# Christina-hshi/SH-assembly

Hardware: AMD Instinct MI355X
Metric: k-mers counted/sec (whole node), CQF build, C.elegans-like k=47 (higher is better)
Workload: dtype u64

## Files before the change

sh-assembly_amd/csrc/kmer_kernels.hip:

```cpp
#include "shk_device.h"

#define SHK_SEED_A 0x3c8bfbb395c60474ULL
#define SHK_SEED_C 0x3193c18562a02b4cULL
#define SHK_SEED_G 0x20323ed082572324ULL
#define SHK_SEED_T 0x295549f54be24456ULL
#define SHK_HASH_WAVES 4
#define SHK_MAX_K 191
#define SHK_MAX_READ 65535

__device__ __forceinline__ uint64_t shk_seed_fwd(unsigned c) {
  const unsigned u = c & 0xDF;
  return (u == 'A' || c == 4) ? SHK_SEED_A : (u == 'C' || c == 7) ? SHK_SEED_C : (u == 'G' || c == 3) ? SHK_SEED_G : (u == 'T' || c == 1) ? SHK_SEED_T : 0ULL;
}
__device__ __forceinline__ uint64_t shk_seed_rc(unsigned c) {
  c &= 7;
  return c == 1 ? SHK_SEED_T : c == 3 ? SHK_SEED_G : c == 7 ? SHK_SEED_C : c == 4 ? SHK_SEED_A : 0ULL;
}

__device__ __forceinline__ uint32_t shk_nl_flags(uint32_t w) {
  uint32_t x = w ^ 0x0A0A0A0Au;
  return ~(((x & 0x7F7F7F7Fu) + 0x7F7F7F7Fu) | x | 0x7F7F7F7Fu);
}

__device__ __forceinline__ uint4 shk_unit_flags(const uint8_t *text, uint64_t a0, uint64_t u, uint64_t off,
                                                uint64_t end) {
  const uint4 v = *reinterpret_cast<const uint4 *>(text + a0 + 16 * u);
  uint32_t w[4] = {v.x, v.y, v.z, v.w};
  uint64_t b0 = a0 + 16 * u;
#pragma unroll
  for (int i = 0; i < 4; i++) {
    uint32_t f = shk_nl_flags(w[i]);
    uint64_t wb = b0 + 4 * i;
    if (wb < off || wb + 4 > end) {
#pragma unroll
      for (int j = 0; j < 4; j++)
        if (wb + j < off || wb + j >= end) f &= ~(0x80u << (8 * j));
    }
    w[i] = f;
  }
  return make_uint4(w[0], w[1], w[2], w[3]);
}

#define SHK_PARSE_SEGS 16
__device__ __forceinline__ void shk_segment_units(uint64_t nunits, unsigned seg, uint64_t *u0, uint64_t *u1) {
  const uint64_t per = (nunits + SHK_PARSE_SEGS - 1) / SHK_PARSE_SEGS;
  *u0 = per * seg < nunits ? per * seg : nunits;
  *u1 = *u0 + per < nunits ? *u0 + per : nunits;
}

__global__ void k_count_lines(const uint8_t *text, const uint64_t *chunk_off, const uint64_t *chunk_len,
                              uint64_t *nlines_seg) {
  __shared__ uint64_t scratch[SHK_MAX_WAVES + 1];
  const unsigned c = blockIdx.x / SHK_PARSE_SEGS, seg = blockIdx.x % SHK_PARSE_SEGS;
  const uint64_t off = chunk_off[c], end = off + chunk_len[c];
  const uint64_t a0 = off & ~15ULL;
  const uint64_t nunits = (end - a0 + 15) / 16;
  uint64_t u0, u1;
  shk_segment_units(nunits, seg, &u0, &u1);
  uint64_t cnt = 0;
  for (uint64_t u = u0 + threadIdx.x; u < u1; u += blockDim.x) {
    uint4 f = shk_unit_flags(text, a0, u, off, end);
    cnt += __popc(f.x) + __popc(f.y) + __popc(f.z) + __popc(f.w);
  }
  uint64_t tot = shk_block_sum64(cnt, scratch);
  if (threadIdx.x == 0) nlines_seg[blockIdx.x] = tot;
}

__global__ void k_scan_chunks(uint64_t *nlines_seg, unsigned nchunks, uint64_t *reads_base, uint64_t *nreads_total) {
  __shared__ uint64_t scratch[SHK_MAX_WAVES + 1];
  __shared__ uint64_t carry_s;
  if (threadIdx.x == 0) carry_s = 0;
  __syncthreads();
  for (unsigned base = 0; base < nchunks; base += blockDim.x) {
    unsigned c = base + threadIdx.x;
    uint64_t nl = 0;
    if (c < nchunks)
      for (unsigned sg = 0; sg < SHK_PARSE_SEGS; sg++) {
        const uint64_t v = nlines_seg[(uint64_t)c * SHK_PARSE_SEGS + sg];
        nlines_seg[(uint64_t)c * SHK_PARSE_SEGS + sg] = nl;
        nl += v;
      }
    uint64_t v = c < nchunks ? (nl + 2) / 4 : 0;
    uint64_t tot;
    uint64_t ex = shk_block_exscan64(v, &tot, scratch);
    uint64_t carry = carry_s;
    if (c < nchunks) reads_base[c] = carry + ex;
    __syncthreads();
    if (threadIdx.x == 0) carry_s = carry + tot;
    __syncthreads();
  }
  if (threadIdx.x == 0) {
    reads_base[nchunks] = carry_s;
    *nreads_total = carry_s;
  }
}

__global__ void k_emit_reads(const uint8_t *text, const uint64_t *chunk_off, const uint64_t *chunk_len,
                             const uint64_t *reads_base, const uint64_t *line_base_seg, uint64_t *rd_start, uint64_t *rd_end,
                             uint16_t *rd_chunk) {
  __shared__ uint32_t scratch[SHK_MAX_WAVES + 1];
  __shared__ uint64_t line_carry;
  const unsigned c = blockIdx.x / SHK_PARSE_SEGS, seg = blockIdx.x % SHK_PARSE_SEGS;
  const uint64_t off = chunk_off[c], end = off + chunk_len[c];
  const uint64_t a0 = off & ~15ULL;
  const uint64_t nunits = (end - a0 + 15) / 16;
  uint64_t u0, u1;
  shk_segment_units(nunits, seg, &u0, &u1);
  const uint64_t rbase = reads_base[c], nreads = reads_base[c + 1] - rbase;
  if (threadIdx.x == 0) line_carry = line_base_seg[blockIdx.x];
  __syncthreads();
  for (uint64_t ub = u0; ub < u1; ub += blockDim.x) {
    uint64_t u = ub + threadIdx.x;
    uint4 f = make_uint4(0, 0, 0, 0);
    if (u < u1) f = shk_unit_flags(text, a0, u, off, end);
    uint32_t n = __popc(f.x) + __popc(f.y) + __popc(f.z) + __popc(f.w);
    uint32_t tot;
    uint32_t ex = shk_block_exscan(n, &tot, scratch);
    uint64_t line = line_carry + ex;
    if (n) {
      uint32_t w[4] = {f.x, f.y, f.z, f.w};
#pragma unroll
      for (int i = 0; i < 4; i++) {
        uint32_t m = w[i];
        while (m) {
          int bit = __ffs(m) - 1;
          m &= m - 1;
          uint64_t pos = a0 + 16 * u + 4 * i + (bit >> 3);
          uint64_t rd = line >> 2;
          if (rd < nreads) {
            if ((line & 3) == 0) { rd_start[rbase + rd] = pos + 1; rd_chunk[rbase + rd] = (uint16_t)c; }
            else if ((line & 3) == 1) rd_end[rbase + rd] = pos;
          }
          line++;
        }
      }
    }
    __syncthreads();
    if (threadIdx.x == 0) line_carry += tot;
    __syncthreads();
  }
}

__device__ __forceinline__ uint32_t shk_segment_end(const uint8_t *rd, uint32_t len, uint32_t s, uint32_t k) {
  const unsigned lane = shk_lane();
  for (uint32_t base = (s + k) & ~63u; base < len; base += 64) {
    uint32_t pos = base + lane;
    bool isN = pos >= s + k && pos < len && rd[pos] == 'N';
    unsigned long long m = __ballot(isN);
    if (m) return base + (uint32_t)(__ffsll((long long)m) - 1);
  }
  return len;
}

__device__ __forceinline__ void shk_read_bytes(const uint8_t *text, uint64_t st, uint64_t en, unsigned lane, uint32_t c[4]) {
  const uint64_t len = en > st ? en - st : 0;
#pragma unroll
  for (int t = 0; t < 4; t++) {
    const uint32_t pos = (uint32_t)t * 64 + lane;
    c[t] = pos < len ? text[st + pos] : 0u;
  }
}
__device__ __forceinline__ void shk_read_masks(const uint32_t c[4], unsigned long long nm[4]) {
#pragma unroll
  for (int t = 0; t < 4; t++) nm[t] = __ballot(c[t] == 'N');
}
__device__ __forceinline__ uint32_t shk_segment_end_pre(const unsigned long long nm[4], const uint8_t *rd, uint32_t len,
                                                        uint32_t s, uint32_t k) {
  if (len > 256) return shk_segment_end(rd, len, s, k);
  const uint32_t from = s + k;
#pragma unroll
  for (int t = 0; t < 4; t++) {
    if ((uint32_t)t < (from >> 6)) continue;
    unsigned long long m = nm[t];
    if ((uint32_t)t == (from >> 6)) m &= ~0ULL << (from & 63);
    if (m) return (uint32_t)t * 64 + (uint32_t)(__ffsll((long long)m) - 1);
  }
  return len;
}

__device__ __forceinline__ uint32_t shk_bytes_below(uint32_t n) { return n >= 4 ? 0xFFFFFFFFu : ((1u << (8 * n)) - 1u); }
__global__ void k_count_keys(const uint8_t *text, const uint64_t *rd_start, const uint64_t *rd_end,
                             const uint64_t *nreads_p, uint32_t k, uint32_t *nkeys, uint32_t *err) {
  const uint64_t nreads = *nreads_p;
  const uint64_t stride = (uint64_t)gridDim.x * blockDim.x;
  for (uint64_t r = (uint64_t)blockIdx.x * blockDim.x + threadIdx.x; r < nreads; r += stride) {
    const uint64_t st = rd_start[r], en = rd_end[r];
    uint32_t cnt = 0;
    if (en - st > SHK_MAX_READ) atomicOr(err, SHK_E_BAD_FASTQ);
    else if (en - st >= k) {
      const uint32_t len = (uint32_t)(en - st);
      const uint8_t *rd = text + st;
      const uint64_t a = st + k, e = en;
      uint32_t any = 0;
      for (uint64_t u = a & ~15ULL; u < e; u += 16) {
        const uint4 v = *reinterpret_cast<const uint4 *>(text + u);
        const uint32_t w[4] = {v.x, v.y, v.z, v.w};
#pragma unroll
        for (int i = 0; i < 4; i++) {
          const uint64_t b = u + 4 * i;
          const uint32_t lo = a > b ? (uint32_t)(a - b > 4 ? 4 : a - b) : 0u;
          const uint32_t hi = e > b ? (uint32_t)(e - b > 4 ? 4 : e - b) : 0u;
          const uint32_t valid = shk_bytes_below(hi) & ~shk_bytes_below(lo);
          const uint32_t x = (w[i] ^ 0x4E4E4E4Eu) | ~valid;
          any |= (x - 0x01010101u) & ~x & 0x80808080u;
        }
      }
      if (!any) cnt = len - k + 1;
      else {
        uint32_t s0 = 0;
        while (len >= s0 + k) {
          uint32_t e0 = s0 + k;
          while (e0 < len && rd[e0] != 'N') e0++;
          cnt += e0 - s0 - k + 1;
          if (e0 == len) break;
          s0 = e0 + 1;
        }
      }
    }
    nkeys[r] = cnt;
  }
}

__global__ void k_hash_reads(const uint8_t *text, const uint64_t *rd_start, const uint64_t *rd_end,
// ... 101 lines not shown
```

sh-assembly_amd/csrc/shk_api.hip:

```cpp
#include "../../include/shk.h"
#include <thread>

#include <hip/hip_runtime.h>
#include <math.h>
#include <stdio.h>
#include <stdlib.h>
#include <string.h>
#include <vector>
#include <string>
#include <algorithm>
#include <unordered_set>
#include <unordered_map>

#include "kmer_kernels.hip"
#include "roll_kernels.hip"
#include "partition_kernels.hip"
#include "cqf_kernels.hip"
#include "merge2_kernels.hip"
#include "walk_kernels.hip"
#include "unitig_kernels.hip"

#define SHK_SLACK 256

enum {
  KP_COUNT_LINES, KP_SCAN_CHUNKS, KP_EMIT_READS, KP_COUNT_KEYS, KP_HASH, KP_SCAN, KP_RP_PREP, KP_RP_HIST,
  KP_RP_SCATTER, KP_MERGE_SUM, KP_REGION_SCAN, KP_MERGE_WRITE, KP_MERGE_SPILL, KP_PLACE, KP_MARKS, KP_LOOKUP, KP_WALK, KP_UG_WALK, KP_UG_FINISH, KP_MERGE_FUSED, KP_MERGE_SAMPLE, KP_MISC, KP_ROLL_HIST, KP_ROLL_SCATTER, KP_PACK, KP_RP_SLOTS, KP_RP_SCATTER_NARROW, KP_SPECTRUM, KP_JOIN, KP_N
};
static const char *kp_names[KP_N] = {
  "k_count_lines", "k_scan_chunks", "k_emit_reads", "k_count_keys", "k_hash_reads", "k_scan_*", "k_rp_prep",
  "k_rp_hist", "k_rp_scatter", "k_region_merge<summary>", "k_region_scan", "k_region_merge<write>",
  "k_region_merge<spill>", "k_region_place", "k_denoise_marks", "k_lookup", "k_extend_forward+k_select_seeds", "k_ug_walk", "k_ug_check/emit/median/links", "k_region_merge<fused>", "k_region_merge<sample>", "misc", "k_roll_hist", "k_roll_scatter", "k_pack_reads", "k_rp_slot_cursors", "k_rp_scatter<narrow>", "k_region_spectrum", "k_region_join"};

struct PendingEvent { int id; hipEvent_t a, b; };

#define SHK_SCALAR_WORDS 64
enum ShkDevSlot {
  DS_NREADS = 0,
  DS_NWORDS = 1,
  DS_SCAN_TOTAL = 2,
  DS_MARKS = 3,
  DS_MAX_COUNT = 4,
  DS_DUMP_STOP = 5,
  DS_JOIN_STOP = 6,
  DS_JOIN_ACC = 7,
  DS_WALK_IN = 8,
  DS_WALK_OUT = 10,
  DS_SPECTRUM = 12,
  DS_STAMPS = 16,
  DS_PAIR_LEN = 40,
  DS_PAIR_BASE = 42,
  DS_EXTENT = 46,
  DS_END = 48
};
enum ShkHostSlot {
  HP_COUNTERS = 0,
  HP_SPECTRUM = 8,
  HP_ERR = 40,
  HP_NREADS = 41,
  HP_NWORDS = 42,
  HP_NWORDS_IN = 43,
  HP_FREE_PTR = 44,
  HP_TOTAL = 45,
  HP_AUX = 46,
  HP_MARKS = 47,
  HP_IFIN = 48,
  HP_IFIRST = 49,
  HP_WALK_IN = 50,
  HP_WALK_OUT = 52,
  HP_PAIR = 56,
  HP_END = 62
};
enum { CNT_NEWD, CNT_ADDED, CNT_REMOVED, CNT_ADDED_BEFORE };
static_assert(HP_COUNTERS + SHK_NCOUNTERS <= HP_ERR, "the counters mirror ends before the error word");
static_assert(HP_COUNTERS + SHK_NCOUNTERS <= HP_SPECTRUM && DS_SPECTRUM + (int)SHK_SPEC_WORDS <= DS_STAMPS, "the spectrum's totals have four words of their own");
static_assert(DS_END <= SHK_SCALAR_WORDS && HP_END <= SHK_SCALAR_WORDS, "both blocks fit their 64 words");
static_assert(DS_PAIR_BASE + 4 == DS_EXTENT && HP_PAIR + (DS_EXTENT - DS_PAIR_LEN) == HP_END, "the pair block is uploaded in one copy");

enum { RP_SCATTER_GROUPED, RP_SCATTER_WIDE, RP_SCATTER_TILE };
struct ShkPartLevel {
  uint8_t scatter;
  bool pair_hist;
  bool may_slot;
  bool may_narrow;
};

struct ShkStageBufs {
  hipStream_t stream = hipStream_t();
  bool lent = false;
  uint8_t *d_text = nullptr;
  uint64_t *d_chunk_off = nullptr, *d_chunk_len = nullptr, *d_nlines = nullptr, *d_reads_base = nullptr;
  uint64_t *d_rd_start = nullptr, *d_rd_end = nullptr;
  uint16_t *d_rd_chunk = nullptr;
  uint32_t *d_nkeys = nullptr;
  uint64_t *d_key_base = nullptr;
  uint64_t *d_words[2] = {};
  uint64_t *d_scalars = nullptr;
  uint64_t *d_block_sums = nullptr;
  uint64_t *d_hist[4] = {};
  uint64_t *d_base_sub = nullptr;
  uint64_t *d_base[5] = {};
  uint64_t *d_cursor = nullptr;
  uint64_t *d_end[3] = {};
  uint32_t *d_tfb = nullptr;
  uint32_t *d_err = nullptr;
  uint64_t *h_pinned = nullptr;
  uint32_t last_err_bits = 0;
  uint32_t region_cap = 0;
  uint32_t slot_overflows = 0;
  int slots_off = 0;
  uint64_t roll_cap = 0;
  uint32_t up_overflows = 0;
  int up_off = 0;
  double prof_ms[KP_N] = {};
  uint64_t prof_n[KP_N] = {};
  std::vector<PendingEvent> pending;
  std::vector<hipEvent_t> evpool;
};

struct shk_ctx : ShkStageBufs {
  shk_config cfg;
  int dev;
  uint64_t g_nslots;
  uint64_t q_lo, nslots, xnslots, nblocks, table_bytes;
  uint32_t nregions, rbits;
  uint32_t nlevels;
  ShkRpLevel lv[4];
  ShkPartLevel part[4];
  bool roll_two;
  bool roll_slots;
  uint32_t threads, hash_groups;
  uint64_t nelts, ndistinct;
  uint32_t rounds_left, rounds_done;
  uint8_t *tab[2];
  uint64_t *fin[2];
  int cur;
  uint8_t *d_up[2];
  hipStream_t copy_stream;
  hipEvent_t up_done[2];
  int up_next, up_pending[2];
  uint32_t *d_summary;
  long long *d_tile_a, *d_tile_b, *d_tile_f;
  uint64_t *d_dump_offs;
  int big_image;
  uint8_t *spill[2];
  int live;
  int rec_live;
  int table_stale;
  int lazy_ok;
  int foreign_marks;
  uint32_t *d_over_list;
  int spill_valid; const uint64_t *spill_words; uint32_t spill_lo, spill_hi; int spill_denoise, spill_big;
  uint64_t spill_nover;
  uint16_t *d_newchunks;
  unsigned long long *d_chist;
  uint64_t *h_chist;
  uint32_t chist_n;
  uint32_t sample_stride;
  uint32_t pt_lo, pt_split, pt_hi; int pt_valid; uint64_t pt_nprot;
  const uint64_t *pt_words;
  unsigned long long *d_counters;
  uint64_t max_reads;
  int prof_on;
  double new_frac;
  int staged;
  uint32_t *d_isum; uint8_t *d_ilens; uint64_t *d_fin_i; uint64_t *d_prot;
  int counted;
  uint64_t *d_send[2];
  int send_next;
  struct ShkFront *front;
};

#define HIPCHK(x) do { hipError_t e_ = (x); if (e_ != hipSuccess) { fprintf(stderr, "libshk: %s failed: %s (%s:%d)\n", #x, hipGetErrorString(e_), __FILE__, __LINE__); return SHK_ERR_HIP; } } while (0)

static hipEvent_t ev_get(ShkStageBufs *c) {
  if (!c->evpool.empty()) { hipEvent_t e = c->evpool.back(); c->evpool.pop_back(); return e; }
  hipEvent_t e; hipEventCreate(&e); return e;
}
struct ProfScope {
  ShkStageBufs *c; int id; bool on; hipEvent_t a, b;
  ProfScope(const shk_ctx *ctx, ShkStageBufs *c_, int id_) : c(c_), id(id_), on(ctx->prof_on != 0) {
    if (on) { a = ev_get(c); b = ev_get(c); hipEventRecord(a, c->stream); }
  }
  ProfScope(shk_ctx *ctx, int id_) : ProfScope(ctx, ctx, id_) {}
  ~ProfScope() {
    if (on) { hipEventRecord(b, c->stream); PendingEvent p = {id, a, b}; c->pending.push_back(p); }
  }
};
static void prof_collect(ShkStageBufs *c) {
  for (size_t i = 0; i < c->pending.size(); i++) {
    float ms = 0;
    hipEventSynchronize(c->pending[i].b);
    hipEventElapsedTime(&ms, c->pending[i].a, c->pending[i].b);
    c->prof_ms[c->pending[i].id] += ms;
    c->prof_n[c->pending[i].id]++;
    c->evpool.push_back(c->pending[i].a);
    c->evpool.push_back(c->pending[i].b);
  }
  c->pending.clear();
}

static int map_err_bits(uint32_t bits) {
  if (!bits) return SHK_OK;
  if (bits & SHK_E_TABLE_FULL) return SHK_ERR_TABLE_FULL;
  if (bits & (SHK_E_OLD_EXTENT | SHK_E_NEW_EXTENT | SHK_E_HASH_FULL | SHK_E_RUN_TOO_LONG)) return SHK_ERR_REGION;
  if (bits & SHK_E_CORRUPT) return SHK_ERR_CORRUPT;
  if (bits & SHK_E_BAD_FASTQ) return SHK_ERR_FASTQ;
  if (bits & SHK_E_KEYS_FULL) return SHK_ERR_BATCH;
  return SHK_ERR_CORRUPT;
}

extern "C" const char *shk_strerror(int code) {
  switch (code) {
    case SHK_OK: return "ok";
    case SHK_ERR_ARG: return "bad argument or unsupported geometry";
    case SHK_ERR_HIP: return "HIP runtime error (is a GPU present?)";
    case SHK_ERR_TABLE_FULL: return "counting quotient filter is full";
    case SHK_ERR_REGION: return "a 256-quotient region exceeds the kernel's on-chip image or hash";
    case SHK_ERR_CORRUPT: return "table metadata inconsistent or key outside this context's range";
    case SHK_ERR_FASTQ: return "malformed FASTQ input";
    case SHK_ERR_BATCH: return "batch exceeds the capacities given to shk_create";
    case SHK_ERR_IO: return "file I/O error";
  }
  return "unknown error";
}
extern "C" uint32_t shk_last_error_bits(shk_ctx *c) { return c ? c->last_err_bits : 0; }

template <typename T> static int dmalloc(T **p, uint64_t n) {
  void *v = nullptr;
  HIPCHK(hipMalloc(&v, n * sizeof(T) + SHK_SLACK));
  *p = (T *)v;
  return 0;
}

static int ensure_chist(shk_ctx *c);
static int point_alloc(shk_ctx *c);
static uint64_t level_out(const shk_ctx *c, uint32_t l) { return (uint64_t)c->lv[l].nbuckets << c->lv[l].bits; }

static uint64_t words_cap(const shk_ctx *c) { return c->cfg.max_batch_keys + (c->roll_slots ? c->cfg.max_batch_keys / 64 : 0); }

static int bufs_alloc(const shk_ctx *c, ShkStageBufs *b, bool lent) {
  const uint64_t capk = c->cfg.max_batch_keys;
  const uint32_t maxch = SHK_MAX_CHUNKS;
  b->lent = lent;
  if (lent) HIPCHK(hipStreamCreateWithFlags(&b->stream, hipStreamNonBlocking));
  else HIPCHK(hipStreamCreate(&b->stream));
  if (dmalloc(&b->d_text, c->cfg.max_batch_bytes + 64)) return SHK_ERR_HIP;
  if (dmalloc(&b->d_chunk_off, maxch) || dmalloc(&b->d_chunk_len, maxch) || dmalloc(&b->d_nlines, (uint64_t)maxch * SHK_PARSE_SEGS) ||
      dmalloc(&b->d_reads_base, maxch + 1)) return SHK_ERR_HIP;
  if (dmalloc(&b->d_rd_start, c->max_reads + 1) || dmalloc(&b->d_rd_end, c->max_reads + 1) ||
      dmalloc(&b->d_nkeys, c->max_reads + 1) || dmalloc(&b->d_rd_chunk, c->max_reads + 1) || dmalloc(&b->d_key_base, c->max_reads + 2)) return SHK_ERR_HIP;
  if (!lent && (dmalloc(&b->d_words[0], words_cap(c) + 1) || dmalloc(&b->d_words[1], words_cap(c) + 1))) return SHK_ERR_HIP;
  if (dmalloc(&b->d_scalars, SHK_SCALAR_WORDS)) return SHK_ERR_HIP;
  HIPCHK(hipMemsetAsync(b->d_scalars, 0, SHK_SCALAR_WORDS * 8, b->stream));
  {
    uint64_t mx = capk > c->max_reads ? capk : c->max_reads;
    uint64_t pw = 1ULL << c->rbits;
    if (pw > mx) mx = pw;
    if (dmalloc(&b->d_block_sums, mx / SHK_SCAN_TILE + 4 + 8192)) return SHK_ERR_HIP;
  }
  if (dmalloc(&b->d_base[0], 2)) return SHK_ERR_HIP;
  for (uint32_t l = 0; l < c->nlevels; l++) {
    const uint64_t n = level_out(c, l);
    if (dmalloc(&b->d_hist[l], (n << c->lv[l].ng_log2) + 1)) return SHK_ERR_HIP;
    if (!(lent && l + 1 == c->nlevels) && dmalloc(&b->d_base[l + 1], n + 2)) return SHK_ERR_HIP;
    if (l == 0 && dmalloc(&b->d_base_sub, (n << c->lv[0].ng_log2) + 2)) return SHK_ERR_HIP;
  }
  { const uint64_t nb = level_out(c, c->nlevels - 1), first = 1ULL << (c->lv[0].bits + c->lv[0].ng_log2);
    if (dmalloc(&b->d_cursor, (nb > first ? nb : first) + 2)) return SHK_ERR_HIP; }
  if (dmalloc(&b->d_tfb, (c->roll_slots ? 2 * words_cap(c) : capk) / SHK_RP_TILE + 2)) return SHK_ERR_HIP;
  if (c->roll_slots && (dmalloc(&b->d_end[1], level_out(c, 0) + 2) || dmalloc(&b->d_end[2], level_out(c, 1) + 2))) return SHK_ERR_HIP;
  if (dmalloc(&b->d_err, 4)) return SHK_ERR_HIP;
  HIPCHK(hipMemsetAsync(b->d_err, 0, 16, b->stream));
  HIPCHK(hipHostMalloc((void **)&b->h_pinned, SHK_SCALAR_WORDS * sizeof(uint64_t), hipHostMallocDefault));
  HIPCHK(hipStreamSynchronize(b->stream));
  return SHK_OK;
}

static void bufs_free(const shk_ctx *c, ShkStageBufs *b) {
  if (b->stream) hipStreamSynchronize(b->stream);
  prof_collect(b);
  for (size_t i = 0; i < b->evpool.size(); i++) hipEventDestroy(b->evpool[i]);
  b->evpool.clear();
  hipFree(b->d_text); hipFree(b->d_chunk_off); hipFree(b->d_chunk_len); hipFree(b->d_nlines); hipFree(b->d_reads_base);
  hipFree(b->d_rd_start); hipFree(b->d_rd_end); hipFree(b->d_rd_chunk); hipFree(b->d_nkeys); hipFree(b->d_key_base); hipFree(b->d_scalars);
  hipFree(b->d_block_sums); hipFree(b->d_base_sub); hipFree(b->d_cursor); hipFree(b->d_end[1]); hipFree(b->d_end[2]); hipFree(b->d_tfb); hipFree(b->d_err);
  if (!b->lent) { hipFree(b->d_words[0]); hipFree(b->d_words[1]); }
  for (uint32_t l = 0; l < 4; l++) hipFree(b->d_hist[l]);
  for (uint32_t l = 0; l < 5; l++) if (!(b->lent && l == c->nlevels)) hipFree(b->d_base[l]);
  hipHostFree(b->h_pinned);
  if (b->stream) hipStreamDestroy(b->stream);
  *b = ShkStageBufs();
}

static int create_init(shk_ctx *c, const shk_config *cfg) {
  const uint32_t ns = cfg->num_shards ? cfg->num_shards : 1;
  c->cfg = *cfg;
  c->dev = cfg->device;
  HIPCHK(hipSetDevice(c->dev));
  c->g_nslots = 1ULL << cfg->qb;
  if (c->g_nslots / ns < 64) return SHK_ERR_ARG;
  c->nslots = c->g_nslots / ns;
  c->q_lo = c->nslots * cfg->shard_index;
  c->xnslots = c->nslots + (uint64_t)(10 * sqrt((double)c->g_nslots));
  c->nblocks = (c->xnslots + 63) / 64;
  c->table_bytes = c->nblocks * SHK_BLOCK_BYTES;
  c->nregions = (uint32_t)((c->nslots + SHK_REGION - 1) / SHK_REGION);
  c->rbits = 0;
  while ((1u << c->rbits) < c->nregions) c->rbits++;
  const uint32_t mlb = cfg->max_level_bits ? cfg->max_level_bits : 10;
  if (mlb > 10) return SHK_ERR_ARG;
  const uint32_t nlevels = (c->rbits + mlb - 1) / mlb;
  if (nlevels > 4) return SHK_ERR_ARG;
  c->nlevels = nlevels ? nlevels : 1;
  {
    uint32_t left = c->rbits, nb = 1;
    for (uint32_t l = 0; l < c->nlevels; l++) {
      uint32_t bits = (left + (c->nlevels - l) - 1) / (c->nlevels - l);
      left -= bits;
      c->lv[l].shift = left; c->lv[l].bits = bits; c->lv[l].nbuckets = nb; c->lv[l].hb = cfg->hb; c->lv[l].q_lo = c->q_lo;
      c->lv[l].nslots = c->nslots; c->lv[l].cb = 0; c->lv[l].out32 = 0; c->lv[l].ablate = 0; c->lv[l].ng_log2 = 0; c->lv[l].slot_cap = 0;
      nb <<= bits;
    }
    c->lv[c->nlevels - 1].out32 = 1;
    if (c->lv[0].bits >= 2 && c->lv[0].bits <= 7 && !getenv("SHK_RP_NO_GROUPS")) c->lv[0].ng_log2 = 3;
  }
  c->threads = cfg->threads_per_group ? cfg->threads_per_group : 512;
  if (c->threads < 64 || c->threads > 1024 || (c->threads & (c->threads - 1))) return SHK_ERR_ARG;
  c->hash_groups = cfg->hash_groups ? cfg->hash_groups : 2048;
  const bool words8 = getenv("SHK_RP_WORDS8") && atoi(getenv("SHK_RP_WORDS8")) != 0;
  c->roll_two = c->nlevels >= 2 && c->lv[0].bits + c->lv[1].bits <= 14;
  for (uint32_t l = 0; l < c->nlevels; l++) {
    const bool last = l + 1 == c->nlevels;
    c->part[l].scatter = l == 0 && c->lv[0].ng_log2 ? RP_SCATTER_GROUPED : c->threads >= 512 && !last && c->lv[l].bits <= 8 ? RP_SCATTER_WIDE : RP_SCATTER_TILE;
    c->part[l].pair_hist = l == 0 && c->roll_two && c->lv[1].ng_log2 == 0;
    c->part[l].may_slot = last && l >= 1 && c->lv[l].out32;
    c->part[l].may_narrow = l >= 1 && l + 2 == c->nlevels && !words8;
    c->lv[l].cb = 32 - 16 - c->lv[c->nlevels - 1].bits;
  }
  c->roll_slots = c->nlevels == 3 && c->part[1].may_narrow && c->part[2].may_slot &&
                  !(getenv("SHK_ROLL_SLOTS") && atoi(getenv("SHK_ROLL_SLOTS")) == 0) &&
                  cfg->max_batch_keys / (level_out(c, 1)) >= 28800;
  c->rounds_left = cfg->num_denoise;
  c->max_reads = cfg->max_batch_reads ? cfg->max_batch_reads : cfg->max_batch_bytes / 16 + 1024;
  { int rc = bufs_alloc(c, c, false); if (rc) return rc; }
  for (int i = 0; i < 2; i++) {
    if (dmalloc(&c->tab[i], c->table_bytes)) return SHK_ERR_HIP;
    if (dmalloc(&c->fin[i], (uint64_t)c->nregions + 2)) return SHK_ERR_HIP;
  }
  if (dmalloc(&c->d_summary, SHK_SUM_STRIDE * (uint64_t)c->nregions + 8)) return SHK_ERR_HIP;
  if (dmalloc(&c->d_dump_offs, (uint64_t)c->nregions + 2)) return SHK_ERR_HIP;
  c->sample_stride = c->nregions >= (1u << 20) ? 16 : 8;
  if (const char *e = getenv("SHK_SAMPLE_STRIDE")) c->sample_stride = (uint32_t)atoi(e);
  else if (c->nregions < (1u << 14)) c->sample_stride = 0;
  c->lazy_ok = 1;
  c->foreign_marks = 0;
  if (const char *e = getenv("SHK_LAZY_PLACE")) c->lazy_ok = atoi(e) != 0;
  if (dmalloc(&c->spill[0], (uint64_t)c->nregions * SHK_SPILL_STRIDE) || dmalloc(&c->d_over_list, (uint64_t)c->nregions + 1)) return SHK_ERR_HIP;
  { uint64_t nt = c->nregions / SHK_RSCAN_TILE + 2;
    if (dmalloc(&c->d_tile_a, nt) || dmalloc(&c->d_tile_b, nt) || dmalloc(&c->d_tile_f, nt)) return SHK_ERR_HIP; }
  if (dmalloc(&c->d_counters, SHK_NCOUNTERS)) return SHK_ERR_HIP;
  HIPCHK(hipMemsetAsync(c->tab[0], 0, c->table_bytes + SHK_SLACK, c->stream));
  HIPCHK(hipMemsetAsync(c->tab[1], 0, c->table_bytes + SHK_SLACK, c->stream));
  HIPCHK(hipMemsetAsync(c->fin[0], 0, ((uint64_t)c->nregions + 2) * 8, c->stream));
  HIPCHK(hipMemsetAsync(c->fin[1], 0, ((uint64_t)c->nregions + 2) * 8, c->stream));
  HIPCHK(hipStreamSynchronize(c->stream));
  if (cfg->num_denoise > 0 || cfg->num_shards > 1) {
    if (ensure_chist(c) || point_alloc(c)) return SHK_ERR_HIP;
  }
  if (cfg->num_shards > 1) {
    for (int b = 0; b < 2; b++)
      if (dmalloc(&c->d_send[b], c->cfg.max_batch_keys + 1)) return SHK_ERR_HIP;
  }
  return SHK_OK;
}

extern "C" int shk_create(const shk_config *cfg, shk_ctx **out) {
  if (!cfg || !out) return SHK_ERR_ARG;
  if (cfg->qb < 6 || cfg->qb > 40 || cfg->hb != cfg->qb + 8 || cfg->k < 1 || cfg->k > SHK_MAX_K) return SHK_ERR_ARG;
  uint32_t ns = cfg->num_shards ? cfg->num_shards : 1;
  if (ns & (ns - 1)) return SHK_ERR_ARG;
  if (cfg->shard_index >= ns) return SHK_ERR_ARG;
  if (cfg->hb + SHK_CHUNK_BITS > 64) return SHK_ERR_ARG;
  shk_ctx *c = new shk_ctx();
  const int rc = create_init(c, cfg);
  if (rc) { shk_destroy(c); return rc; }
  *out = c;
  return SHK_OK;
}

static void front_destroy(shk_ctx *c);
extern "C" void shk_destroy(shk_ctx *c) {
  if (!c) return;
  hipSetDevice(c->dev);
  front_destroy(c);
  if (c->stream) hipStreamSynchronize(c->stream);
  if (c->copy_stream) {
    hipStreamSynchronize(c->copy_stream);
    for (int b = 0; b < 2; b++) { if (c->d_up[b]) hipFree(c->d_up[b]); if (c->up_done[b]) hipEventDestroy(c->up_done[b]); }
    hipStreamDestroy(c->copy_stream);
  }
  if (getenv("SHK_STAMPS") && c->d_scalars) {
    unsigned long long st[16];
    hipMemcpy(st, c->d_scalars + DS_STAMPS, sizeof(st), hipMemcpyDeviceToHost);
    static const char *nm[9] = {"stage+init", "fold keys", "old rank/select", "count sort", "merge pass", "scan+stats", "(unused)", "placement", "stores"};
    unsigned long long tot = 0; for (int i = 0; i < 9; i++) tot += st[i];
    for (int i = 0; i < 9; i++) fprintf(stderr, "SHK_STAMPS %-16s %6.2f %%\n", nm[i], tot ? 100.0 * st[i] / tot : 0.0);
  }
  for (int i = 0; i < 2; i++) { hipFree(c->tab[i]); hipFree(c->fin[i]); hipFree(c->d_send[i]); }
  hipFree(c->d_isum); hipFree(c->d_ilens); hipFree(c->d_fin_i); hipFree(c->d_prot);
  hipFree(c->d_newchunks); hipFree(c->d_chist); hipHostFree(c->h_chist);
  hipFree(c->spill[0]); hipFree(c->spill[1]); hipFree(c->d_over_list); hipFree(c->d_summary); hipFree(c->d_dump_offs); hipFree(c->d_tile_a); hipFree(c->d_tile_b); hipFree(c->d_tile_f); hipFree(c->d_counters);
  bufs_free(c, c);
  delete c;
}

template <typename T>
static int run_scan(const shk_ctx *c, ShkStageBufs *b, const T *in, uint64_t n_max, const uint64_t *n_dev, uint64_t *out, uint64_t *sums = nullptr) {
  ProfScope ps(c, b, KP_SCAN);
  if (!sums) sums = b->d_block_sums;
  const uint32_t nb = (uint32_t)(n_max / SHK_SCAN_TILE + 1);
  hipLaunchKernelGGL((k_scan_reduce<T>), dim3(nb), dim3(c->threads), 0, b->stream, in, n_max, n_dev, sums);
  hipLaunchKernelGGL(k_scan_top, dim3(1), dim3(c->threads), 0, b->stream, sums, (uint64_t)nb, b->d_scalars + DS_SCAN_TOTAL);
  hipLaunchKernelGGL((k_scan_apply<T>), dim3(nb), dim3(c->threads), 0, b->stream, in, n_max, n_dev, sums,
                     b->d_scalars + DS_SCAN_TOTAL, out);
  HIPCHK(hipGetLastError());
  return 0;
}

static int err_enqueue(ShkStageBufs *b) { HIPCHK(hipMemcpyAsync(b->h_pinned + HP_ERR, b->d_err, 4, hipMemcpyDeviceToHost, b->stream)); return 0; }
static int err_take(ShkStageBufs *b, bool record, uint32_t *bits) {
  *bits = *(uint32_t *)(b->h_pinned + HP_ERR);
  if (*bits && record) b->last_err_bits = *bits;
  if (*bits) HIPCHK(hipMemsetAsync(b->d_err, 0, 16, b->stream));
  return 0;
}
static int fetch_err(ShkStageBufs *b, uint32_t *bits) {
  if (err_enqueue(b)) return SHK_ERR_HIP;
  HIPCHK(hipStreamSynchronize(b->stream));
  return err_take(b, true, bits);
}
static int set_nwords(ShkStageBufs *b, uint64_t n) {
  b->h_pinned[HP_NWORDS_IN] = n;
  HIPCHK(hipMemcpyAsync(b->d_scalars + DS_NWORDS, b->h_pinned + HP_NWORDS_IN, 8, hipMemcpyHostToDevice, b->stream));
  return 0;
}

static int upload_wait(shk_ctx *c, const void *text, int on_device, hipStream_t stream) {
  for (int u = 0; on_device && u < 2; u++)
    if (c->d_up[u] && text == (const void *)c->d_up[u] && c->up_pending[u]) { HIPCHK(hipStreamWaitEvent(stream, c->up_done[u], 0)); c->up_pending[u] = 0; }
  return SHK_OK;
}

static bool chunk_labels_ok(uint32_t nchunks, uint32_t chunk_first, uint32_t chunk_mul) {
  return nchunks != 0 && nchunks <= SHK_MAX_CHUNKS && chunk_first + (uint64_t)(nchunks - 1) * chunk_mul < SHK_MAX_CHUNKS;
}

static bool text_aligned(const void *text, int on_device) { return !on_device || ((uintptr_t)text & 15) == 0; }
static int parse_stage(const shk_ctx *c, ShkStageBufs *b, const void *text, int on_device, uint64_t text_bytes, const uint64_t *chunk_off,
                       const uint64_t *chunk_len, uint32_t nchunks, const uint8_t **dtext_out, uint64_t *nreads_out) {
  if (!text_aligned(text, on_device)) return SHK_ERR_ARG;
  for (uint32_t i = 0; i < nchunks; i++)
    if (chunk_off[i] + chunk_len[i] > text_bytes) return SHK_ERR_ARG;
  const uint8_t *dtext;
  if (on_device) {
    dtext = (const uint8_t *)text;
  } else {
    if (text_bytes > c->cfg.max_batch_bytes) return SHK_ERR_BATCH;
    HIPCHK(hipMemcpyAsync(b->d_text, text, text_bytes, hipMemcpyHostToDevice, b->stream));
    dtext = b->d_text;
  }
  HIPCHK(hipMemcpyAsync(b->d_chunk_off, chunk_off, nchunks * 8, hipMemcpyHostToDevice, b->stream));
  HIPCHK(hipMemcpyAsync(b->d_chunk_len, chunk_len, nchunks * 8, hipMemcpyHostToDevice, b->stream));
  { ProfScope ps(c, b, KP_COUNT_LINES);
    hipLaunchKernelGGL(k_count_lines, dim3(nchunks * SHK_PARSE_SEGS), dim3(c->threads), 0, b->stream, dtext, b->d_chunk_off, b->d_chunk_len, b->d_nlines); }
  { ProfScope ps(c, b, KP_SCAN_CHUNKS);
    hipLaunchKernelGGL(k_scan_chunks, dim3(1), dim3(c->threads), 0, b->stream, b->d_nlines, nchunks, b->d_reads_base, b->d_scalars + DS_NREADS); }
  HIPCHK(hipMemcpyAsync(b->h_pinned + HP_NREADS, b->d_scalars + DS_NREADS, 8, hipMemcpyDeviceToHost, b->stream));
  HIPCHK(hipStreamSynchronize(b->stream));
  const uint64_t nreads = b->h_pinned[HP_NREADS];
  if (nreads > c->max_reads) return SHK_ERR_BATCH;
  { ProfScope ps(c, b, KP_EMIT_READS);
    hipLaunchKernelGGL(k_emit_reads, dim3(nchunks * SHK_PARSE_SEGS), dim3(c->threads), 0, b->stream, dtext, b->d_chunk_off, b->d_chunk_len,
                       b->d_reads_base, b->d_nlines, b->d_rd_start, b->d_rd_end, b->d_rd_chunk); }
  *dtext_out = dtext;
  *nreads_out = nreads;
  return SHK_OK;
}

static int hash_stage(const shk_ctx *c, ShkStageBufs *b, const void *text, int on_device, uint64_t text_bytes, const uint64_t *chunk_off,
                      const uint64_t *chunk_len, uint32_t nchunks, uint32_t chunk_first, uint32_t chunk_mul, bool hist0 = false) {
  if (!chunk_labels_ok(nchunks, chunk_first, chunk_mul)) return SHK_ERR_BATCH;
  if (!text_aligned(text, on_device)) return SHK_ERR_ARG;
  if (hist0) HIPCHK(hipMemsetAsync(b->d_hist[0], 0, (1ULL << (c->lv[0].bits + c->lv[0].ng_log2)) * 8, b->stream));
  const uint8_t *dtext;
  uint64_t nreads;
  { int rc = parse_stage(c, b, text, on_device, text_bytes, chunk_off, chunk_len, nchunks, &dtext, &nreads); if (rc) return rc; }
  uint32_t groups = c->hash_groups;
  { uint64_t need = nreads / (c->threads / SHK_WAVE) + 1; if (need < groups) groups = (uint32_t)need; }
  { ProfScope ps(c, b, KP_COUNT_KEYS);
    const uint64_t blocks = nreads / 256 + 1;
    hipLaunchKernelGGL(k_count_keys, dim3((uint32_t)(blocks < (1u << 20) ? blocks : (1u << 20))), dim3(256), 0, b->stream, dtext, b->d_rd_start, b->d_rd_end,
                       b->d_scalars + DS_NREADS, c->cfg.k, b->d_nkeys, b->d_err); }
  if (run_scan<uint32_t>(c, b, b->d_nkeys, nreads, nullptr, b->d_key_base)) return SHK_ERR_HIP;
  HIPCHK(hipMemcpyAsync(b->d_scalars + DS_NWORDS, b->d_key_base + nreads, 8, hipMemcpyDeviceToDevice, b->stream));
  { ProfScope ps(c, b, KP_HASH);
    const uint32_t ht = c->threads < SHK_HASH_WAVES * SHK_WAVE ? c->threads : SHK_HASH_WAVES * SHK_WAVE;
    hipLaunchKernelGGL(k_hash_reads, dim3(groups * (c->threads / ht)), dim3(ht), 0, b->stream, dtext, b->d_rd_start, b->d_rd_end,
                       b->d_scalars + DS_NREADS, b->d_rd_chunk, chunk_first, chunk_mul, b->d_key_base, c->cfg.k, c->cfg.hb,
                       b->d_words[0], c->cfg.max_batch_keys, b->d_err, hist0 ? b->d_hist[0] : nullptr, c->lv[0].shift, c->lv[0].bits, c->q_lo, c->lv[0].ng_log2); }
  HIPCHK(hipGetLastError());
  return SHK_OK;
}

static int pack_stage(const shk_ctx *c, ShkStageBufs *b, ShkRollArgs &A, uint64_t nreads, uint64_t text_bytes, uint64_t *buf) {
  A.pk = nullptr; A.pk_base = nullptr; A.pk_flag = nullptr;
  const uint64_t cap_units = c->cfg.max_batch_keys / 2 > 1 ? c->cfg.max_batch_keys / 2 - 1 : 0;
  if (getenv("SHK_NO_PACK") || text_bytes / 64 + nreads + 1 > cap_units) return SHK_OK;
  ProfScope ps(c, b, KP_PACK);
  const uint32_t t = c->threads < 256 ? c->threads : 256;
  { const uint64_t blocks = nreads / t + 1;
    hipLaunchKernelGGL(k_pack_count, dim3((uint32_t)(blocks < 4096 ? blocks : 4096)), dim3(t), 0, b->stream, (const uint64_t *)b->d_rd_start,
                       (const uint64_t *)b->d_rd_end, (const uint64_t *)(b->d_scalars + DS_NREADS), c->cfg.k, b->d_nkeys); }
  if (run_scan<uint32_t>(c, b, b->d_nkeys, nreads, nullptr, b->d_key_base)) return SHK_ERR_HIP;
  { const uint64_t blocks = nreads * 4 / t + 1;
    hipLaunchKernelGGL(k_pack_reads, dim3((uint32_t)(blocks < 16384 ? blocks : 16384)), dim3(t), 0, b->stream, A.text, A.safe_end,
                       (const uint64_t *)b->d_rd_start, (const uint64_t *)b->d_rd_end, (const uint64_t *)(b->d_scalars + DS_NREADS),
                       (const uint64_t *)b->d_key_base, b->d_nkeys, (ShkQuad *)buf, cap_units); }
  A.pk = (const ShkQuad *)buf; A.pk_base = b->d_key_base; A.pk_flag = b->d_nkeys;
  return SHK_OK;
}

static void roll_args(const shk_ctx *c, ShkStageBufs *b, ShkRollArgs &A, const uint8_t *dtext, uint64_t text_bytes,
                      uint32_t chunk_first, uint32_t chunk_mul) {
  A.text = dtext; A.safe_end = (text_bytes + 15) & ~15ULL;
  A.rd_start = b->d_rd_start; A.rd_end = b->d_rd_end; A.nreads_p = b->d_scalars + DS_NREADS; A.rd_chunk = b->d_rd_chunk;
  A.chunk_first = chunk_first; A.chunk_mul = chunk_mul; A.k = c->cfg.k; A.hb = c->cfg.hb;
  A.cap = c->cfg.max_batch_keys; A.err = b->d_err;
}
static void launch_roll_hist(const shk_ctx *c, ShkStageBufs *b, const ShkRollArgs &A, uint64_t nreads, bool wide) {
  const bool small = c->threads < 512;
  const uint32_t t = small ? 64 : wide ? 512 : 256, max_blocks = small ? 64 : wide ? 1024 : 4096;
  const uint64_t blocks = nreads / t + 1;
  const dim3 grid((uint32_t)(blocks < max_blocks ? blocks : max_blocks));
  if (small && wide) hipLaunchKernelGGL((k_roll_hist<14, 64>), grid, dim3(64), 0, b->stream, A);
  else if (small) hipLaunchKernelGGL((k_roll_hist<10, 64>), grid, dim3(64), 0, b->stream, A);
  else if (wide) hipLaunchKernelGGL((k_roll_hist<14, 512>), grid, dim3(512), 0, b->stream, A);
  else hipLaunchKernelGGL((k_roll_hist<10, 256>), grid, dim3(256), 0, b->stream, A);
}
static void launch_roll_scatter(const shk_ctx *c, ShkStageBufs *b, const ShkRollArgs &A, uint64_t nreads) {
  ProfScope ps(c, b, KP_ROLL_SCATTER);
  if (c->threads >= 512) {
    const uint64_t blocks = nreads / 1024 + 1;
    hipLaunchKernelGGL((k_roll_scatter<1024, 1>), dim3((uint32_t)(blocks < 512 ? blocks : 512)), dim3(1024), 0, b->stream, A);
  } else {
    const uint64_t blocks = nreads / 64 + 1;
    hipLaunchKernelGGL((k_roll_scatter<64, 4>), dim3((uint32_t)(blocks < 64 ? blocks : 64)), dim3(64), 0, b->stream, A);
  }
}

static bool roll_path(const shk_ctx *c) { return c->nlevels >= 2; }

static uint64_t up_slot_capacity(double m, uint64_t unit) {
  const uint64_t cp = (uint64_t)ceil(m + 6.0 * sqrt(8.0 * m + 1.0) + 16.0);
  return (cp + unit - 1) / unit * unit;
}
// ... 2405 lines not shown
```

Measured before the change: 35.78 billion.

## Cache newline bitmask in count pass and emit reads from mask

The line-counting kernel now writes a 16-bit newline bitmask per 16-byte text unit. The read-emission kernel then scans this compact mask, 128 bytes of text per thread, instead of rereading and re-classifying the whole text. This cuts the second pass's memory traffic by about 8x and gives each thread more work per block scan, with fewer barriers. The cost is an extra write pass of text/8 bytes and an extra buffer, reallocated with a stream sync if it is too small.

```diff
diff --git a/sh-assembly_amd/csrc/kmer_kernels.hip b/sh-assembly_amd/csrc/kmer_kernels.hip
--- a/sh-assembly_amd/csrc/kmer_kernels.hip
+++ b/sh-assembly_amd/csrc/kmer_kernels.hip
@@ -22,24 +22,25 @@
   return ~(((x & 0x7F7F7F7Fu) + 0x7F7F7F7Fu) | x | 0x7F7F7F7Fu);
 }
 
+__device__ __forceinline__ void shk_clip_flags(uint32_t w[4], uint64_t b0, uint64_t off, uint64_t end) {
+#pragma unroll
+  for (int i = 0; i < 4; i++) {
+    uint64_t wb = b0 + 4 * i;
+    if (wb < off || wb + 4 > end) {
+#pragma unroll
+      for (int j = 0; j < 4; j++)
+        if (wb + j < off || wb + j >= end) w[i] &= ~(0x80u << (8 * j));
+    }
+  }
+}
 __device__ __forceinline__ uint4 shk_unit_flags(const uint8_t *text, uint64_t a0, uint64_t u, uint64_t off,
                                                 uint64_t end) {
   const uint4 v = *reinterpret_cast<const uint4 *>(text + a0 + 16 * u);
-  uint32_t w[4] = {v.x, v.y, v.z, v.w};
-  uint64_t b0 = a0 + 16 * u;
-#pragma unroll
-  for (int i = 0; i < 4; i++) {
-    uint32_t f = shk_nl_flags(w[i]);
-    uint64_t wb = b0 + 4 * i;
-    if (wb < off || wb + 4 > end) {
-#pragma unroll
-      for (int j = 0; j < 4; j++)
-        if (wb + j < off || wb + j >= end) f &= ~(0x80u << (8 * j));
-    }
-    w[i] = f;
-  }
+  uint32_t w[4] = {shk_nl_flags(v.x), shk_nl_flags(v.y), shk_nl_flags(v.z), shk_nl_flags(v.w)};
+  shk_clip_flags(w, a0 + 16 * u, off, end);
   return make_uint4(w[0], w[1], w[2], w[3]);
 }
+__device__ __forceinline__ uint32_t shk_flags_to_bits(uint32_t f) { return ((f >> 7) * 0x01020408u) >> 24; }
 
 #define SHK_PARSE_SEGS 16
 __device__ __forceinline__ void shk_segment_units(uint64_t nunits, unsigned seg, uint64_t *u0, uint64_t *u1) {
@@ -49,7 +50,7 @@
 }
 
 __global__ void k_count_lines(const uint8_t *text, const uint64_t *chunk_off, const uint64_t *chunk_len,
-                              uint64_t *nlines_seg) {
+                              uint64_t *nlines_seg, uint16_t *nlmask) {
   __shared__ uint64_t scratch[SHK_MAX_WAVES + 1];
   const unsigned c = blockIdx.x / SHK_PARSE_SEGS, seg = blockIdx.x % SHK_PARSE_SEGS;
   const uint64_t off = chunk_off[c], end = off + chunk_len[c];
@@ -59,8 +60,14 @@
   shk_segment_units(nunits, seg, &u0, &u1);
   uint64_t cnt = 0;
   for (uint64_t u = u0 + threadIdx.x; u < u1; u += blockDim.x) {
-    uint4 f = shk_unit_flags(text, a0, u, off, end);
-    cnt += __popc(f.x) + __popc(f.y) + __popc(f.z) + __popc(f.w);
+    const uint64_t b0 = a0 + 16 * u;
+    const uint4 v = *reinterpret_cast<const uint4 *>(text + b0);
+    uint32_t w[4] = {shk_nl_flags(v.x), shk_nl_flags(v.y), shk_nl_flags(v.z), shk_nl_flags(v.w)};
+    if (nlmask)
+      nlmask[b0 >> 4] = (uint16_t)(shk_flags_to_bits(w[0]) | shk_flags_to_bits(w[1]) << 4 | shk_flags_to_bits(w[2]) << 8 |
+                                   shk_flags_to_bits(w[3]) << 12);
+    shk_clip_flags(w, b0, off, end);
+    cnt += __popc(w[0]) + __popc(w[1]) + __popc(w[2]) + __popc(w[3]);
   }
   uint64_t tot = shk_block_sum64(cnt, scratch);
   if (threadIdx.x == 0) nlines_seg[blockIdx.x] = tot;
@@ -95,19 +102,20 @@
   }
 }
 
-__global__ void k_emit_reads(const uint8_t *text, const uint64_t *chunk_off, const uint64_t *chunk_len,
-                             const uint64_t *reads_base, const uint64_t *line_base_seg, uint64_t *rd_start, uint64_t *rd_end,
-                             uint16_t *rd_chunk) {
-  __shared__ uint32_t scratch[SHK_MAX_WAVES + 1];
-  __shared__ uint64_t line_carry;
-  const unsigned c = blockIdx.x / SHK_PARSE_SEGS, seg = blockIdx.x % SHK_PARSE_SEGS;
-  const uint64_t off = chunk_off[c], end = off + chunk_len[c];
+__device__ __forceinline__ void shk_emit_line(uint64_t line, uint64_t pos, unsigned c, uint64_t rbase, uint64_t nreads,
+                                              uint64_t *rd_start, uint64_t *rd_end, uint16_t *rd_chunk) {
+  const uint64_t rd = line >> 2;
+  if (rd < nreads) {
+    if ((line & 3) == 0) { rd_start[rbase + rd] = pos + 1; rd_chunk[rbase + rd] = (uint16_t)c; }
+    else if ((line & 3) == 1) rd_end[rbase + rd] = pos;
+  }
+}
+
+__device__ __forceinline__ void shk_emit_from_text(const uint8_t *text, unsigned c, uint64_t off, uint64_t end, uint64_t u0, uint64_t u1,
+                                                   uint64_t line0, uint64_t rbase, uint64_t nreads, uint64_t *rd_start,
+                                                   uint64_t *rd_end, uint16_t *rd_chunk, uint32_t *scratch, uint64_t *line_carry) {
   const uint64_t a0 = off & ~15ULL;
-  const uint64_t nunits = (end - a0 + 15) / 16;
-  uint64_t u0, u1;
-  shk_segment_units(nunits, seg, &u0, &u1);
-  const uint64_t rbase = reads_base[c], nreads = reads_base[c + 1] - rbase;
-  if (threadIdx.x == 0) line_carry = line_base_seg[blockIdx.x];
+  if (threadIdx.x == 0) *line_carry = line0;
   __syncthreads();
   for (uint64_t ub = u0; ub < u1; ub += blockDim.x) {
     uint64_t u = ub + threadIdx.x;
@@ -116,7 +124,7 @@
     uint32_t n = __popc(f.x) + __popc(f.y) + __popc(f.z) + __popc(f.w);
     uint32_t tot;
     uint32_t ex = shk_block_exscan(n, &tot, scratch);
-    uint64_t line = line_carry + ex;
+    uint64_t line = *line_carry + ex;
     if (n) {
       uint32_t w[4] = {f.x, f.y, f.z, f.w};
 #pragma unroll
@@ -125,20 +133,73 @@
         while (m) {
           int bit = __ffs(m) - 1;
           m &= m - 1;
-          uint64_t pos = a0 + 16 * u + 4 * i + (bit >> 3);
-          uint64_t rd = line >> 2;
-          if (rd < nreads) {
-            if ((line & 3) == 0) { rd_start[rbase + rd] = pos + 1; rd_chunk[rbase + rd] = (uint16_t)c; }
-            else if ((line & 3) == 1) rd_end[rbase + rd] = pos;
-          }
-          line++;
-        }
-      }
-    }
-    __syncthreads();
-    if (threadIdx.x == 0) line_carry += tot;
-    __syncthreads();
-  }
+          shk_emit_line(line++, a0 + 16 * u + 4 * i + (bit >> 3), c, rbase, nreads, rd_start, rd_end, rd_chunk);
+        }
+      }
+    }
+    __syncthreads();
+    if (threadIdx.x == 0) *line_carry += tot;
+    __syncthreads();
+  }
+}
+
+__device__ __forceinline__ void shk_emit_from_flags(const uint16_t *nlmask, unsigned c, uint64_t off, uint64_t end, uint64_t u0, uint64_t u1,
+                                                    uint64_t line0, uint64_t rbase, uint64_t nreads, uint64_t *rd_start,
+                                                    uint64_t *rd_end, uint16_t *rd_chunk, uint32_t *scratch) {
+  if (u0 >= u1) return;
+  const uint64_t a0 = off & ~15ULL;
+  const uint64_t lo = u0 ? a0 + 16 * u0 : off;
+  const uint64_t hi = a0 + 16 * u1 < end ? a0 + 16 * u1 : end;
+  const uint64_t stride = (uint64_t)blockDim.x * 128;
+  for (uint64_t gb = (lo & ~127ULL); gb < hi; gb += stride) {
+    const uint64_t g = gb + (uint64_t)threadIdx.x * 128;
+    uint32_t w[4] = {0, 0, 0, 0};
+    if (g < hi) {
+      const uint4 v = *reinterpret_cast<const uint4 *>(nlmask + (g >> 4));
+      w[0] = v.x; w[1] = v.y; w[2] = v.z; w[3] = v.w;
+      if (g < lo || g + 128 > hi) {
+#pragma unroll
+        for (int i = 0; i < 4; i++) {
+          const uint64_t wb = g + 32 * i;
+          const uint32_t below_lo = wb >= lo ? 0u : lo - wb >= 32 ? 0xFFFFFFFFu : (1u << (uint32_t)(lo - wb)) - 1u;
+          const uint32_t below_hi = wb >= hi ? 0u : hi - wb >= 32 ? 0xFFFFFFFFu : (1u << (uint32_t)(hi - wb)) - 1u;
+          w[i] &= below_hi & ~below_lo;
+        }
+      }
+    }
+    const uint32_t n = __popc(w[0]) + __popc(w[1]) + __popc(w[2]) + __popc(w[3]);
+    uint32_t tot;
+    const uint32_t ex = shk_block_exscan(n, &tot, scratch);
+    uint64_t line = line0 + ex;
+    if (n) {
+#pragma unroll
+      for (int i = 0; i < 4; i++) {
+        uint32_t m = w[i];
+        while (m) {
+          const int bit = __ffs(m) - 1;
+          m &= m - 1;
+          shk_emit_line(line++, g + 32 * i + bit, c, rbase, nreads, rd_start, rd_end, rd_chunk);
+        }
+      }
+    }
+    line0 += tot;
+  }
+}
+
+__global__ void k_emit_reads(const uint8_t *text, const uint16_t *nlmask, const uint64_t *chunk_off, const uint64_t *chunk_len,
+                             const uint64_t *reads_base, const uint64_t *line_base_seg, uint64_t *rd_start, uint64_t *rd_end,
+                             uint16_t *rd_chunk) {
+  __shared__ uint32_t scratch[SHK_MAX_WAVES + 1];
+  __shared__ uint64_t line_carry;
+  const unsigned c = blockIdx.x / SHK_PARSE_SEGS, seg = blockIdx.x % SHK_PARSE_SEGS;
+  const uint64_t off = chunk_off[c], end = off + chunk_len[c];
+  const uint64_t nunits = (end - (off & ~15ULL) + 15) / 16;
+  uint64_t u0, u1;
+  shk_segment_units(nunits, seg, &u0, &u1);
+  const uint64_t rbase = reads_base[c], nreads = reads_base[c + 1] - rbase;
+  const uint64_t line0 = line_base_seg[blockIdx.x];
+  if (nlmask) shk_emit_from_flags(nlmask, c, off, end, u0, u1, line0, rbase, nreads, rd_start, rd_end, rd_chunk, scratch);
+  else shk_emit_from_text(text, c, off, end, u0, u1, line0, rbase, nreads, rd_start, rd_end, rd_chunk, scratch, &line_carry);
 }
 
 __device__ __forceinline__ uint32_t shk_segment_end(const uint8_t *rd, uint32_t len, uint32_t s, uint32_t k) {
diff --git a/sh-assembly_amd/csrc/shk_api.hip b/sh-assembly_amd/csrc/shk_api.hip
--- a/sh-assembly_amd/csrc/shk_api.hip
+++ b/sh-assembly_amd/csrc/shk_api.hip
@@ -91,6 +91,8 @@
   uint64_t *d_chunk_off = nullptr, *d_chunk_len = nullptr, *d_nlines = nullptr, *d_reads_base = nullptr;
   uint64_t *d_rd_start = nullptr, *d_rd_end = nullptr;
   uint16_t *d_rd_chunk = nullptr;
+  uint16_t *d_nlmask = nullptr;
+  uint64_t nlmask_units = 0;
   uint32_t *d_nkeys = nullptr;
   uint64_t *d_key_base = nullptr;
   uint64_t *d_words[2] = {};
@@ -128,6 +130,7 @@
   ShkPartLevel part[4];
   bool roll_two;
   bool roll_slots;
+  bool parse_mask;
   uint32_t threads, hash_groups;
   uint64_t nelts, ndistinct;
   uint32_t rounds_left, rounds_done;
@@ -238,6 +241,14 @@
 
 static uint64_t words_cap(const shk_ctx *c) { return c->cfg.max_batch_keys + (c->roll_slots ? c->cfg.max_batch_keys / 64 : 0); }
 
+static int nlmask_alloc(ShkStageBufs *b, uint64_t units) {
+  void *v = nullptr;
+  if (hipMalloc(&v, units * sizeof(uint16_t)) != hipSuccess) { (void)hipGetLastError(); return SHK_ERR_HIP; }
+  b->d_nlmask = (uint16_t *)v;
+  b->nlmask_units = units;
+  return 0;
+}
+
 static int bufs_alloc(const shk_ctx *c, ShkStageBufs *b, bool lent) {
   const uint64_t capk = c->cfg.max_batch_keys;
   const uint32_t maxch = SHK_MAX_CHUNKS;
@@ -245,6 +256,10 @@
   if (lent) HIPCHK(hipStreamCreateWithFlags(&b->stream, hipStreamNonBlocking));
   else HIPCHK(hipStreamCreate(&b->stream));
   if (dmalloc(&b->d_text, c->cfg.max_batch_bytes + 64)) return SHK_ERR_HIP;
+  if (c->parse_mask) {
+    const uint64_t tb = c->cfg.max_batch_bytes > 4 * capk ? c->cfg.max_batch_bytes : 4 * capk;
+    if (nlmask_alloc(b, tb / 16 + 8)) return SHK_ERR_HIP;
+  }
   if (dmalloc(&b->d_chunk_off, maxch) || dmalloc(&b->d_chunk_len, maxch) || dmalloc(&b->d_nlines, (uint64_t)maxch * SHK_PARSE_SEGS) ||
       dmalloc(&b->d_reads_base, maxch + 1)) return SHK_ERR_HIP;
   if (dmalloc(&b->d_rd_start, c->max_reads + 1) || dmalloc(&b->d_rd_end, c->max_reads + 1) ||
@@ -282,6 +297,7 @@
   for (size_t i = 0; i < b->evpool.size(); i++) hipEventDestroy(b->evpool[i]);
   b->evpool.clear();
   hipFree(b->d_text); hipFree(b->d_chunk_off); hipFree(b->d_chunk_len); hipFree(b->d_nlines); hipFree(b->d_reads_base);
+  hipFree(b->d_nlmask);
   hipFree(b->d_rd_start); hipFree(b->d_rd_end); hipFree(b->d_rd_chunk); hipFree(b->d_nkeys); hipFree(b->d_key_base); hipFree(b->d_scalars);
   hipFree(b->d_block_sums); hipFree(b->d_base_sub); hipFree(b->d_cursor); hipFree(b->d_end[1]); hipFree(b->d_end[2]); hipFree(b->d_tfb); hipFree(b->d_err);
   if (!b->lent) { hipFree(b->d_words[0]); hipFree(b->d_words[1]); }
@@ -340,6 +356,7 @@
   c->roll_slots = c->nlevels == 3 && c->part[1].may_narrow && c->part[2].may_slot &&
                   !(getenv("SHK_ROLL_SLOTS") && atoi(getenv("SHK_ROLL_SLOTS")) == 0) &&
                   cfg->max_batch_keys / (level_out(c, 1)) >= 28800;
+  c->parse_mask = !(getenv("SHK_PARSE_MASK") && atoi(getenv("SHK_PARSE_MASK")) == 0);
   c->rounds_left = cfg->num_denoise;
   c->max_reads = cfg->max_batch_reads ? cfg->max_batch_reads : cfg->max_batch_bytes / 16 + 1024;
   { int rc = bufs_alloc(c, c, false); if (rc) return rc; }
@@ -459,20 +476,32 @@
 static int parse_stage(const shk_ctx *c, ShkStageBufs *b, const void *text, int on_device, uint64_t text_bytes, const uint64_t *chunk_off,
                        const uint64_t *chunk_len, uint32_t nchunks, const uint8_t **dtext_out, uint64_t *nreads_out) {
   if (!text_aligned(text, on_device)) return SHK_ERR_ARG;
-  for (uint32_t i = 0; i < nchunks; i++)
+  uint64_t text_end = 0;
+  for (uint32_t i = 0; i < nchunks; i++) {
     if (chunk_off[i] + chunk_len[i] > text_bytes) return SHK_ERR_ARG;
+    if (chunk_off[i] + chunk_len[i] > text_end) text_end = chunk_off[i] + chunk_len[i];
+  }
+  if (!on_device && text_bytes > c->cfg.max_batch_bytes) return SHK_ERR_BATCH;
+  const uint64_t mask_units = text_end / 16 + 8;
+  if (c->parse_mask && mask_units > b->nlmask_units) {
+    HIPCHK(hipStreamSynchronize(b->stream));
+    hipFree(b->d_nlmask);
+    b->d_nlmask = nullptr;
+    b->nlmask_units = 0;
+    (void)nlmask_alloc(b, mask_units);
+  }
+  uint16_t *const nlmask = c->parse_mask && mask_units <= b->nlmask_units ? b->d_nlmask : nullptr;
   const uint8_t *dtext;
   if (on_device) {
     dtext = (const uint8_t *)text;
   } else {
-    if (text_bytes > c->cfg.max_batch_bytes) return SHK_ERR_BATCH;
     HIPCHK(hipMemcpyAsync(b->d_text, text, text_bytes, hipMemcpyHostToDevice, b->stream));
     dtext = b->d_text;
   }
   HIPCHK(hipMemcpyAsync(b->d_chunk_off, chunk_off, nchunks * 8, hipMemcpyHostToDevice, b->stream));
   HIPCHK(hipMemcpyAsync(b->d_chunk_len, chunk_len, nchunks * 8, hipMemcpyHostToDevice, b->stream));
   { ProfScope ps(c, b, KP_COUNT_LINES);
-    hipLaunchKernelGGL(k_count_lines, dim3(nchunks * SHK_PARSE_SEGS), dim3(c->threads), 0, b->stream, dtext, b->d_chunk_off, b->d_chunk_len, b->d_nlines); }
+    hipLaunchKernelGGL(k_count_lines, dim3(nchunks * SHK_PARSE_SEGS), dim3(c->threads), 0, b->stream, dtext, b->d_chunk_off, b->d_chunk_len, b->d_nlines, nlmask); }
   { ProfScope ps(c, b, KP_SCAN_CHUNKS);
     hipLaunchKernelGGL(k_scan_chunks, dim3(1), dim3(c->threads), 0, b->stream, b->d_nlines, nchunks, b->d_reads_base, b->d_scalars + DS_NREADS); }
   HIPCHK(hipMemcpyAsync(b->h_pinned + HP_NREADS, b->d_scalars + DS_NREADS, 8, hipMemcpyDeviceToHost, b->stream));
@@ -480,7 +509,7 @@
   const uint64_t nreads = b->h_pinned[HP_NREADS];
   if (nreads > c->max_reads) return SHK_ERR_BATCH;
   { ProfScope ps(c, b, KP_EMIT_READS);
-    hipLaunchKernelGGL(k_emit_reads, dim3(nchunks * SHK_PARSE_SEGS), dim3(c->threads), 0, b->stream, dtext, b->d_chunk_off, b->d_chunk_len,
+    hipLaunchKernelGGL(k_emit_reads, dim3(nchunks * SHK_PARSE_SEGS), dim3(c->threads), 0, b->stream, dtext, (const uint16_t *)nlmask, b->d_chunk_off, b->d_chunk_len,
                        b->d_reads_base, b->d_nlines, b->d_rd_start, b->d_rd_end, b->d_rd_chunk); }
   *dtext_out = dtext;
   *nreads_out = nreads;
```

Measured after the change: 37.49 billion, median of 6. 4.8% higher.
